# ShuangXieIrene/ssds.pytorch

Measured on AMD Instinct MI355X. Metric: images/sec (fwd+decode+NMS) SSD-MobileNetV2@512, higher is better.
Workload: dtype bf16

## Files before the change

ssds.pytorch_amd/csrc/ssdk_flow_common.h:

```cpp
#pragma once
#include "ssdk_common.h"

namespace ssdk {

typedef __bf16 fl_bf16x8 __attribute__((ext_vector_type(8)));
typedef _Float16 fl_f16x8 __attribute__((ext_vector_type(8)));
typedef float f32x4 __attribute__((ext_vector_type(4)));
typedef _Float16 fl_h2 __attribute__((ext_vector_type(2)));

struct FlowParams {
  const u16* x;
  u16* y;
  const u16* we;
  const float* se;
  const float* be;
  const u16* wd;
  const u16* bd;
  const u16* wp;
  const float* sp;
  const float* bp;
  int N, H, W, Cin, Chid, Cout, Ho, Wo, residual;
  int strips, segs, rs;
  int Himg, Wimg, Cimg, layout;
  unsigned long long seg_mask;
  unsigned long long* dbg;
};

template <int DT>
__device__ __forceinline__ f32x4 fl_mfma(const u32x4& a, const u32x4& b, f32x4 c) {
  if constexpr (DT == SSDK_BF16)
    return __builtin_amdgcn_mfma_f32_16x16x32_bf16(__builtin_bit_cast(fl_bf16x8, a), __builtin_bit_cast(fl_bf16x8, b), c, 0, 0, 0);
  else
    return __builtin_amdgcn_mfma_f32_16x16x32_f16(__builtin_bit_cast(fl_f16x8, a), __builtin_bit_cast(fl_f16x8, b), c, 0, 0, 0);
}
__device__ __forceinline__ fl_h2 fl_as_h2(u32 w) { return __builtin_bit_cast(fl_h2, w); }
__device__ __forceinline__ u32 fl_as_u32(fl_h2 v) { return __builtin_bit_cast(u32, v); }
template <int DT> __device__ __forceinline__ u32 fl_to16(float v) {
  if constexpr (DT == SSDK_BF16) {
    u32 b = __builtin_bit_cast(u32, v);
    if ((b & 0x7fffffffu) > 0x7f800000u) return (b >> 16) | 0x40u;
    return (b + 0x7fffu + ((b >> 16) & 1u)) >> 16;
  } else {
    _Float16 h = (_Float16)v;
    return (u32)__builtin_bit_cast(u16, h);
  }
}
typedef float fl_f32x2 __attribute__((ext_vector_type(2)));
typedef __bf16 fl_bf16x2 __attribute__((ext_vector_type(2)));
template <int DT> __device__ __forceinline__ u32 fl_pack2(float a, float b) {
  const fl_f32x2 v = {a, b};
  if constexpr (DT == SSDK_BF16) return __builtin_bit_cast(u32, __builtin_convertvector(v, fl_bf16x2));
  else return __builtin_bit_cast(u32, __builtin_convertvector(v, fl_h2));
}
template <int DT> __device__ __forceinline__ float fl_from16(u32 h) {
  if constexpr (DT == SSDK_BF16) return bf16_bits_to_f32(h);
  else return f16_bits_to_f32(h);
}
__device__ __forceinline__ u32 fl_from_left(u32 v) { return (u32)__builtin_amdgcn_update_dpp(0, (int)v, 0x111, 0xf, 0xf, true); }
__device__ __forceinline__ u32 fl_from_right(u32 v) { return (u32)__builtin_amdgcn_update_dpp(0, (int)v, 0x101, 0xf, 0xf, true); }

typedef float fl_f2 __attribute__((ext_vector_type(2)));
constexpr float kFlSixth = 1.0f / 6.0f;
__device__ __forceinline__ u32 fl_unit_pack(float a, float b, fl_f2 k) {
  const fl_f2 v = {a, b};
  fl_f2 r;
  asm("v_pk_mul_f32 %0, %1, %2 clamp" : "=v"(r) : "v"(v), "v"(k));
  return __builtin_bit_cast(u32, __builtin_amdgcn_cvt_pkrtz(r[0], r[1]));
}
__device__ __forceinline__ fl_h2 fl_fma_clamp01(fl_h2 a, fl_h2 b, fl_h2 c) {
  fl_h2 r;
  asm("v_pk_fma_f16 %0, %1, %2, %3 clamp" : "=v"(r) : "v"(a), "v"(b), "v"(c));
  return r;
}
__device__ __forceinline__ u32 fl_sixth_h2(u32 w) {
  return fl_to16<SSDK_F16>(fl_from16<SSDK_F16>(w & 0xffffu) * kFlSixth) | (fl_to16<SSDK_F16>(fl_from16<SSDK_F16>(w >> 16) * kFlSixth) << 16);
}

}
```

ssds.pytorch_amd/csrc/ssdk_mbflow.hip:

```cpp
#include <stdio.h>
#include <atomic>
#include <type_traits>

#include "ssdk_common.h"
#include "ssdk_flow_common.h"

namespace ssdk {

constexpr int kFlowThreads = 256;

template <int NCH, int NFO>
struct FlowLds {
  static constexpr int T = (NCH + 1) / 2;
  static constexpr int we = 0;
  static constexpr int sb = we + NCH * 1024;
  static constexpr int wd = sb + NCH * 4 * 32;
  static constexpr int bd = wd + NCH * 9 * 4 * 8;
  static constexpr int wp = (bd + NCH * 4 * 8 + 15) & ~15;
  static constexpr int spb = wp + NFO * T * 1024;
  static constexpr int bytes = spb + NFO * 4 * 32;
};

template <int DT, int S, int NCH, int NFO, int NS, bool STEM = false, bool YE = false, bool PAIR = false, bool XD = false>
__global__ __launch_bounds__(kFlowThreads, ((STEM && !YE) || PAIR) ? 3 : 2) void mbflow_kernel(const FlowParams p) {
  static_assert(!PAIR || (S == 1 && !STEM), "row pairs: stride-1 blocks");
  static_assert(!XD || (STEM && !YE), "dword image loads: the stem's interior instance");
  using L = FlowLds<NCH, NFO>;
  constexpr int T = L::T;
  extern __shared__ __attribute__((aligned(16))) unsigned char smem[];
  const u32 tid = threadIdx.x, lane = tid & 63u, wave = tid >> 6;
  const u32 fr = lane & 15u, fg = lane >> 4;
  const int Cin = p.Cin, Chid = p.Chid, Cout = p.Cout;

  for (u32 i = tid; i < (u32)(NCH * 64); i += kFlowThreads) {
    const u32 c = i >> 6, l = i & 63u, hc = c * 16 + (l & 15u), k0 = (l >> 4) * 8;
    u32x4 v = {0u, 0u, 0u, 0u};
    if constexpr (STEM) {
      if (hc < (u32)Chid) {
#pragma unroll
        for (u32 j = 0; j < 8; ++j) {
          u32 ci, ky, kx;
          bool kv;
          if constexpr (XD) {
            const u32 g = k0 >> 3;
            u32 t;
            if (j < 3u) {
              t = 2u * g;
              kx = j == 2u ? 0u : j + 1u;
              kv = true;
            } else if (j < 6u) {
              t = 2u * g + 1u;
              kx = j == 3u ? 0u : j - 3u;
              kv = true;
            } else {
              t = 8u;
              kx = g == 0u ? j - 5u : 0u;
              kv = g == 0u || (g == 1u && j == 7u);
            }
            ci = t / 3u;
            ky = t % 3u;
            kv = kv && ci < (u32)p.Cimg;
          } else {
            const u32 k = k0 + j;
            ci = k / 9u;
            ky = (k % 9u) / 3u;
            kx = k % 3u;
            kv = k < 27u && ci < (u32)p.Cimg;
          }
          const u32 h = kv ? (u32)p.we[(size_t)hc * 96 + (ky * 8 + kx) * 4 + ci] : 0u;
          v[j >> 1] |= h << ((j & 1u) * 16u);
        }
      }
    } else {
      if (hc < (u32)Chid && k0 < (u32)Cin) v = *reinterpret_cast<const u32x4*>(p.we + (size_t)hc * Cin + k0);
    }
    if (hc < (u32)Chid) {
      const float sc = p.se[hc];
      if (sc != 1.0f) {
#pragma unroll
        for (int q = 0; q < 4; ++q) {
          const u32 w2 = v[q];
          v[q] = fl_to16<DT>(fl_from16<DT>(w2 & 0xffffu) * sc) | (fl_to16<DT>(fl_from16<DT>(w2 >> 16) * sc) << 16);
        }
      }
    }
    *reinterpret_cast<u32x4*>(smem + L::we + i * 16) = v;
  }
  for (u32 i = tid; i < (u32)(NCH * 4); i += kFlowThreads) {
    const u32 hc = (i >> 2) * 16 + (i & 3u) * 4;
    f32x4 s = {0.f, 0.f, 0.f, 0.f}, b = {0.f, 0.f, 0.f, 0.f};
    uint2 d = make_uint2(0u, 0u);
    if (hc < (u32)Chid) {
      s = *reinterpret_cast<const f32x4*>(p.se + hc);
      b = *reinterpret_cast<const f32x4*>(p.be + hc);
      d = *reinterpret_cast<const uint2*>(p.bd + hc);
      d = make_uint2(fl_sixth_h2(d.x), fl_sixth_h2(d.y));
    }
    *reinterpret_cast<f32x4*>(smem + L::sb + i * 32) = s;
    *reinterpret_cast<f32x4*>(smem + L::sb + i * 32 + 16) = b;
    *reinterpret_cast<uint2*>(smem + L::bd + i * 8) = d;
  }
  for (u32 i = tid; i < (u32)(NCH * 9 * 4); i += kFlowThreads) {
    const u32 g = i & 3u, tap = (i >> 2) % 9u, c = (i >> 2) / 9u, hc = c * 16 + g * 4;
    uint2 d = make_uint2(0u, 0u);
    if (hc < (u32)Chid) d = *reinterpret_cast<const uint2*>(p.wd + (size_t)tap * Chid + hc);
    *reinterpret_cast<uint2*>(smem + L::wd + i * 8) = d;
  }
  for (u32 i = tid; i < (u32)(NFO * T * 64 * 2); i += kFlowThreads) {
    const u32 half = i & 1u, l = (i >> 1) & 63u, ft = i >> 7, t = ft % (u32)T, f = ft / (u32)T;
    const u32 co = f * 16 + (l & 15u), hc = (2 * t + half) * 16 + (l >> 4) * 4;
    uint2 d = make_uint2(0u, 0u);
    if (co < (u32)Cout && hc < (u32)Chid) d = *reinterpret_cast<const uint2*>(p.wp + (size_t)co * Chid + hc);
    *reinterpret_cast<uint2*>(smem + L::wp + (ft * 64 + l) * 16 + half * 8) = d;
  }
  for (u32 i = tid; i < (u32)(NFO * 4); i += kFlowThreads) {
    const u32 co = (i >> 2) * 16 + (i & 3u) * 4;
    f32x4 s = {0.f, 0.f, 0.f, 0.f}, b = {0.f, 0.f, 0.f, 0.f};
    if (co < (u32)Cout) {
      s = *reinterpret_cast<const f32x4*>(p.sp + co) * 6.0f;
      b = *reinterpret_cast<const f32x4*>(p.bp + co);
    }
    *reinterpret_cast<f32x4*>(smem + L::spb + i * 32) = s;
    *reinterpret_cast<f32x4*>(smem + L::spb + i * 32 + 16) = b;
  }
  __syncthreads();

  const u32 item = blockIdx.x * (kFlowThreads / 64) + (u32)__builtin_amdgcn_readfirstlane((int)wave);
  const int groups = (p.strips + NS - 1) / NS;
  const int nseg = STEM ? __builtin_popcountll(p.seg_mask) : p.segs;
  const u32 per_img = (u32)(groups * nseg);
  if (item >= (u32)p.N * per_img) return;
  const int n = (int)(item / per_img), rem = (int)(item % per_img);
  int seg = rem / groups;
  const int grp = rem % groups;
  if constexpr (STEM) {
    unsigned long long m = p.seg_mask;
    for (int i = 0; i < seg; ++i) m &= m - 1;
    seg = __builtin_ctzll(m);
  }
  constexpr int OW = S == 1 ? 14 : 7;
  constexpr bool MERGE = S == 2 && NS == 2;
  constexpr int NA = MERGE ? 1 : NS;
  const int oy0 = seg * p.rs, oy1 = (oy0 + p.rs < p.Ho ? oy0 + p.rs : p.Ho) - 1;
  int ix[NS], oxl[NA];
  bool col_ok[NS], out_lane[NA];
#pragma unroll
  for (int s = 0; s < NS; ++s) {
    const int strip = grp * NS + s;
    const int ox0 = strip * OW;
    ix[s] = MERGE ? 2 * (grp * 15 + (int)fr) - s : ox0 * S - 1 + (int)fr;
    col_ok[s] = strip < p.strips && (unsigned)ix[s] < (unsigned)p.W;
    if constexpr (!MERGE) {
      oxl[s] = S == 1 ? ox0 + (int)fr - 1 : ox0 + ((int)fr - 1) / 2;
      out_lane[s] = strip < p.strips && (S == 1 ? (fr >= 1u && fr <= 14u) : ((fr & 1u) && fr <= 13u)) && oxl[s] < p.Wo;
    }
  }
  if constexpr (MERGE) {
    oxl[0] = grp * 15 + (int)fr;
    out_lane[0] = fr <= 14u && oxl[0] < p.Wo;
  }

  const u16* ximg = STEM ? p.x + (size_t)n * p.Cimg * p.Himg * p.Wimg : p.x + (size_t)n * p.H * p.W * Cin;
  const bool k_ok = fg * 8u < (u32)Cin;
  constexpr u32 kOOR = 0x40000000u;
  u32 xoff[STEM ? NS : 1][STEM ? 8 : 1], xoff0[(STEM && !YE) ? NS : 1][(STEM && !YE) ? 8 : 1], kyM[STEM ? 3 : 1];
  const int pstr = STEM ? (p.layout == 1 ? 1 : p.Cimg) : 0, cstr = STEM ? (p.layout == 1 ? p.Himg * p.Wimg : 1) : 0;
  if constexpr (STEM) {
    kyM[0] = kyM[1] = kyM[2] = 0u;
#pragma unroll
    for (int j = 0; j < 8; ++j) {
      const u32 k = fg * 8u + (u32)j, ci = k / 9u, ky = (k % 9u) / 3u, kx = k % 3u;
      const bool kv = k < 27u && ci < (u32)p.Cimg;
      const u32 vo = (u32)(2 * (int)fr * pstr + (int)ci * cstr + ((int)ky * p.Wimg + (int)kx) * pstr) * 2u;
      kyM[0] |= (kv && ky == 0u) ? (1u << j) : 0u;
      kyM[1] |= (kv && ky == 1u) ? (1u << j) : 0u;
      kyM[2] |= (kv && ky == 2u) ? (1u << j) : 0u;
#pragma unroll
      for (int s = 0; s < NS; ++s) {
        xoff[s][j] = (kv && col_ok[s] && (unsigned)(2 * ix[s] - 1 + (int)kx) < (unsigned)p.Wimg) ? vo : kOOR;
        if constexpr (!YE) xoff0[s][j] = ky == 0u ? kOOR : xoff[s][j];
      }
    }
  }
  u32 xd_off[XD ? NS : 1][3], xd_off0[XD ? NS : 1][2], xd_edge[2], xd_edge0[2];
  if constexpr (XD) {
    const u32 tA = 2u * fg, tB = 2u * fg + 1u;
    auto voff = [&](u32 t, int shift, int s_) -> u32 {
      const u32 ci = t / 3u, ky = t % 3u;
      const int px = ix[s_] - shift;
      const bool ok = ci < (u32)p.Cimg && grp * NS + s_ < p.strips && (unsigned)px < (unsigned)p.W;
      return ok ? (u32)((2 * (int)fr + (int)ci * p.Himg * p.Wimg + (int)ky * p.Wimg) * 2 + 4 * (1 - shift)) : kOOR;
    };
#pragma unroll
    for (int s = 0; s < NS; ++s) {
      xd_off[s][0] = voff(tA, 0, s);
      xd_off[s][1] = voff(tB, 0, s);
      xd_off[s][2] = fg == 0u ? voff(8u, 0, s) : (fg == 1u ? voff(8u, 1, s) : kOOR);
      xd_off0[s][0] = tA % 3u == 0u ? kOOR : xd_off[s][0];
      xd_off0[s][1] = tB % 3u == 0u ? kOOR : xd_off[s][1];
    }
    xd_edge[0] = fr == 0u ? voff(tA, 1, 0) : kOOR;
    xd_edge[1] = fr == 0u ? voff(tB, 1, 0) : kOOR;
    xd_edge0[0] = tA % 3u == 0u ? kOOR : xd_edge[0];
    xd_edge0[1] = tB % 3u == 0u ? kOOR : xd_edge[1];
  }
  const int xmargin = STEM ? (p.Wimg + 8) * pstr * 2 : 0;
  const __amdgpu_buffer_rsrc_t xrsrc = __builtin_amdgcn_make_buffer_rsrc(
      (void*)(reinterpret_cast<const unsigned char*>(ximg) - xmargin), 0, STEM ? p.Cimg * p.Himg * p.Wimg * 2 + xmargin : 0, 0x00020000);
  constexpr int XW = STEM ? 8 : 4;
  struct XRow {
    u32 w[XW];
  };
  auto load_x = [&](int iy, int s) -> XRow {
    XRow out;
#pragma unroll
    for (int q = 0; q < XW; ++q) out.w[q] = 0u;
    if constexpr (STEM) {
      const int strip = grp * NS + s;
      const int base = ((2 * iy - 1) * p.Wimg + (2 * (strip * 14 - 1) - 1)) * pstr;
      if constexpr (XD) {
        const bool row_in = (unsigned)iy < (unsigned)p.H, top = iy == 0;
        const int soff = row_in ? (base + 1) * 2 + xmargin - 4 : (int)kOOR;
        out.w[0] = (u32)__builtin_amdgcn_raw_buffer_load_b32(xrsrc, (int)(top ? xd_off0[s][0] : xd_off[s][0]), soff, 0);
        out.w[1] = (u32)__builtin_amdgcn_raw_buffer_load_b32(xrsrc, (int)(top ? xd_off0[s][1] : xd_off[s][1]), soff, 0);
        out.w[2] = (u32)__builtin_amdgcn_raw_buffer_load_b32(xrsrc, (int)xd_off[s][2], soff, 0);
        if (s == 0) {
          out.w[3] = (u32)__builtin_amdgcn_raw_buffer_load_b32(xrsrc, (int)(top ? xd_edge0[0] : xd_edge[0]), soff, 0);
          out.w[4] = (u32)__builtin_amdgcn_raw_buffer_load_b32(xrsrc, (int)(top ? xd_edge0[1] : xd_edge[1]), soff, 0);
        }
        return out;
      } else if constexpr (YE) {
        u32 rowmask = 0;
#pragma unroll
        for (int ky = 0; ky < 3; ++ky)
          rowmask |= ((unsigned)iy < (unsigned)p.H && (unsigned)(2 * iy - 1 + ky) < (unsigned)p.Himg) ? kyM[ky] : 0u;
#pragma unroll
        for (int j = 0; j < 8; ++j) {
          const u32 off = (((rowmask >> j) & 1u) && xoff[s][j] != kOOR) ? xoff[s][j] + (u32)(base * 2 + xmargin) : kOOR;
          out.w[j] = (u32)__builtin_amdgcn_raw_buffer_load_b16(xrsrc, (int)off, 0, 0);
        }
      } else {
        const bool row_in = (unsigned)iy < (unsigned)p.H, top = iy == 0;
        const int soff = row_in ? base * 2 + xmargin : (int)kOOR;
#pragma unroll
        for (int j = 0; j < 8; ++j)
          out.w[j] = (u32)__builtin_amdgcn_raw_buffer_load_b16(xrsrc, (int)(top ? xoff0[s][j] : xoff[s][j]), soff, 0);
      }
      return out;
    } else {
      if (k_ok && col_ok[s] && (unsigned)iy < (unsigned)p.H) {
        const u32x4 v = *reinterpret_cast<const u32x4*>(ximg + ((size_t)iy * p.W + ix[s]) * Cin + fg * 8);
        out.w[0] = v[0];
        out.w[1] = v[1];
        out.w[2] = v[2];
        out.w[3] = v[3];
      }
      return out;
    }
  };

  const bool dbgw = p.dbg != nullptr && blockIdx.x == gridDim.x / 2 && __builtin_amdgcn_readfirstlane((int)wave) == 0;
  int dbg_k = 0;
  fl_h2 accA[NA][NCH * 2], accB[NA][NCH * 2], accC[NA][NCH * 2];
  fl_h2 accD[PAIR ? NA : 1][PAIR ? NCH * 2 : 1];

  auto row = [&](const XRow (&xraw)[NS], int iy, auto FINc, auto MIDc, auto INIc, fl_h2 (&fin)[NA][NCH * 2],
                 fl_h2 (&mid)[NA][NCH * 2], fl_h2 (&ini)[NA][NCH * 2], int oy_fin) {
    constexpr bool FIN = decltype(FINc)::value, MID = decltype(MIDc)::value, INI = decltype(INIc)::value;
    if (dbgw && dbg_k < 250) {
      p.dbg[dbg_k++] = __builtin_readcyclecounter();
      if constexpr (STEM) asm volatile("s_waitcnt vmcnt(16)" ::: "memory");
      else asm volatile("s_waitcnt vmcnt(2)" ::: "memory");
      p.dbg[dbg_k++] = __builtin_readcyclecounter();
    }
    u32x4 xf[NS];
#pragma unroll
    for (int s = 0; s < NS; ++s) {
      if constexpr (XD) {
        int oa, ob;
        if (s == 0) {
          oa = (int)xraw[0].w[3];
          ob = (int)xraw[0].w[4];
        } else {
          oa = __builtin_amdgcn_update_dpp(0, (int)xraw[s - 1].w[0], 0x123, 0xf, 0xf, true);
          ob = __builtin_amdgcn_update_dpp(0, (int)xraw[s - 1].w[1], 0x123, 0xf, 0xf, true);
        }
        const u32 an = (u32)__builtin_amdgcn_update_dpp(oa, (int)xraw[s].w[0], 0x111, 0xf, 0xf, false);
        const u32 bn = (u32)__builtin_amdgcn_update_dpp(ob, (int)xraw[s].w[1], 0x111, 0xf, 0xf, false);
        xf[s][0] = xraw[s].w[0];
        xf[s][1] = __builtin_amdgcn_perm(bn, an, 0x07060302u);
        xf[s][2] = xraw[s].w[1];
        xf[s][3] = fg == 1u ? (xraw[s].w[2] & 0xffff0000u) : xraw[s].w[2];
      } else if constexpr (STEM) {
#pragma unroll
        for (int q = 0; q < 4; ++q) xf[s][q] = xraw[s].w[2 * q] | (xraw[s].w[2 * q + 1] << 16);
      } else {
#pragma unroll
        for (int q = 0; q < 4; ++q) xf[s][q] = xraw[s].w[q];
      }
    }
    fl_f2 hi[NS];
#pragma unroll
    for (int s = 0; s < NS; ++s) {
      const float k = (col_ok[s] && (unsigned)iy < (unsigned)p.H) ? kFlSixth : 0.f;
      hi[s] = fl_f2{k, k};
    }
    const bool store_row = FIN && oy_fin >= oy0 && oy_fin <= oy1;
    uint2 resv[NA][NFO];
    if (!STEM && !MERGE && FIN && store_row && p.residual) {
#pragma unroll
      for (int s = 0; s < NA; ++s)
#pragma unroll
        for (int f = 0; f < NFO; ++f) {
          const int co = f * 16 + (int)fg * 4;
          uint2 r = make_uint2(0u, 0u);
          if (out_lane[s] && co < Cout) r = *reinterpret_cast<const uint2*>(ximg + ((size_t)oy_fin * p.W + oxl[s]) * Cin + co);
          resv[s][f] = r;
        }
    }
    asm volatile("" ::: "memory");
    f32x4 e_cur[NS], e_nxt[NS];
    u32x4 wa = *reinterpret_cast<const u32x4*>(smem + L::we + (int)lane * 16);
    {
      const f32x4 bv0 = *reinterpret_cast<const f32x4*>(smem + L::sb + (int)fg * 32 + 16);
#pragma unroll
      for (int s = 0; s < NS; ++s) e_cur[s] = fl_mfma<DT>(wa, xf[s], bv0);
    }
    if (NCH > 1) wa = *reinterpret_cast<const u32x4*>(smem + L::we + (64 + (int)lane) * 16);
#pragma unroll
    for (int c = 0; c < NCH; ++c) {
      asm volatile("" ::: "memory");
      uint2 wt[9];
#pragma unroll
      for (int t = 0; t < 9; ++t) wt[t] = *reinterpret_cast<const uint2*>(smem + L::wd + ((c * 9 + t) * 4 + (int)fg) * 8);
      uint2 bdi = make_uint2(0u, 0u);
      if constexpr (INI) bdi = *reinterpret_cast<const uint2*>(smem + L::bd + (c * 4 + (int)fg) * 8);
      if (c + 1 < NCH) {
        const f32x4 bvn = *reinterpret_cast<const f32x4*>(smem + L::sb + ((c + 1) * 4 + (int)fg) * 32 + 16);
#pragma unroll
        for (int s = 0; s < NS; ++s) e_nxt[s] = fl_mfma<DT>(wa, xf[s], bvn);
        if (c + 2 < NCH) wa = *reinterpret_cast<const u32x4*>(smem + L::we + ((c + 2) * 64 + (int)lane) * 16);
      }
      __builtin_amdgcn_sched_barrier(0);
      u32 ew[NS][2];
#pragma unroll
      for (int s = 0; s < NS; ++s) {
        const f32x4 e = e_cur[s];
        ew[s][0] = fl_unit_pack(e[0], e[1], hi[s]);
        ew[s][1] = fl_unit_pack(e[2], e[3], hi[s]);
      }
      auto fold = [&](fl_h2 l0, fl_h2 l1, fl_h2 c0, fl_h2 c1, fl_h2 r0, fl_h2 r1, int a) {
        auto taps = [&](int ky, fl_h2& a0, fl_h2& a1, bool init) {
          const uint2 w0 = wt[ky * 3], w1 = wt[ky * 3 + 1], w2 = wt[ky * 3 + 2];
          fl_h2 s0 = init ? fl_as_h2(bdi.x) : a0, s1 = init ? fl_as_h2(bdi.y) : a1;
          s0 = __builtin_elementwise_fma(l0, fl_as_h2(w0.x), s0);
          s1 = __builtin_elementwise_fma(l1, fl_as_h2(w0.y), s1);
          s0 = __builtin_elementwise_fma(c0, fl_as_h2(w1.x), s0);
          s1 = __builtin_elementwise_fma(c1, fl_as_h2(w1.y), s1);
          if (ky == 2) {
            s0 = fl_fma_clamp01(r0, fl_as_h2(w2.x), s0);
            s1 = fl_fma_clamp01(r1, fl_as_h2(w2.y), s1);
          } else {
            s0 = __builtin_elementwise_fma(r0, fl_as_h2(w2.x), s0);
            s1 = __builtin_elementwise_fma(r1, fl_as_h2(w2.y), s1);
          }
          asm volatile("" : "+v"(s0), "+v"(s1));
          a0 = s0;
          a1 = s1;
        };
        if constexpr (INI) taps(0, ini[a][2 * c], ini[a][2 * c + 1], true);
        if constexpr (MID) taps(1, mid[a][2 * c], mid[a][2 * c + 1], false);
        if constexpr (FIN) taps(2, fin[a][2 * c], fin[a][2 * c + 1], false);
      };
      if constexpr (MERGE) {
        fold(fl_as_h2(ew[1][0]), fl_as_h2(ew[1][1]), fl_as_h2(ew[0][0]), fl_as_h2(ew[0][1]), fl_as_h2(fl_from_right(ew[1][0])),
             fl_as_h2(fl_from_right(ew[1][1])), 0);
      } else {
#pragma unroll
        for (int s = 0; s < NS; ++s)
          fold(fl_as_h2(fl_from_left(ew[s][0])), fl_as_h2(fl_from_left(ew[s][1])), fl_as_h2(ew[s][0]), fl_as_h2(ew[s][1]),
               fl_as_h2(fl_from_right(ew[s][0])), fl_as_h2(fl_from_right(ew[s][1])), s);
      }
#pragma unroll
      for (int s = 0; s < NS; ++s) e_cur[s] = e_nxt[s];
      __builtin_amdgcn_sched_barrier(0);
    }
    if (dbgw && dbg_k < 250) p.dbg[dbg_k++] = __builtin_readcyclecounter();
    if constexpr (FIN) {
      if (store_row) {
        asm volatile("" ::: "memory");
        f32x4 yacc[NA][NFO];
#pragma unroll
        for (int s = 0; s < NA; ++s)
#pragma unroll
          for (int f = 0; f < NFO; ++f) yacc[s][f] = f32x4{0.f, 0.f, 0.f, 0.f};
#pragma unroll
        for (int t = 0; t < T; ++t) {
          u32x4 db[NA];
#pragma unroll
          for (int s = 0; s < NA; ++s) {
            db[s][0] = fl_as_u32(fin[s][4 * t]);
            db[s][1] = fl_as_u32(fin[s][4 * t + 1]);
            if (2 * t + 1 < NCH) {
              db[s][2] = fl_as_u32(fin[s][(4 * t + 2 < NCH * 2) ? 4 * t + 2 : 0]);
              db[s][3] = fl_as_u32(fin[s][(4 * t + 3 < NCH * 2) ? 4 * t + 3 : 0]);
            } else {
              db[s][2] = 0u;
              db[s][3] = 0u;
            }
          }
#pragma unroll
          for (int f = 0; f < NFO; ++f) {
            const u32x4 wf = *reinterpret_cast<const u32x4*>(smem + L::wp + ((f * T + t) * 64 + (int)lane) * 16);
#pragma unroll
            for (int s = 0; s < NA; ++s) yacc[s][f] = fl_mfma<SSDK_F16>(wf, db[s], yacc[s][f]);
          }
        }
#pragma unroll
        for (int s = 0; s < NA; ++s) {
          if (out_lane[s]) {
            u16* yrow = p.y + (((size_t)n * p.Ho + oy_fin) * p.Wo + oxl[s]) * Cout;
#pragma unroll
            for (int f = 0; f < NFO; ++f) {
              const int co = f * 16 + (int)fg * 4;
              if (co < Cout) {
                const f32x4 spv = *reinterpret_cast<const f32x4*>(smem + L::spb + (f * 4 + (int)fg) * 32);
                const f32x4 bpv = *reinterpret_cast<const f32x4*>(smem + L::spb + (f * 4 + (int)fg) * 32 + 16);
                u32 h01 = fl_pack2<DT>(fmaf(yacc[s][f][0], spv[0], bpv[0]), fmaf(yacc[s][f][1], spv[1], bpv[1]));
                u32 h23 = fl_pack2<DT>(fmaf(yacc[s][f][2], spv[2], bpv[2]), fmaf(yacc[s][f][3], spv[3], bpv[3]));
                if (!STEM && !MERGE && p.residual) {
                  const u32 x01 = resv[s][f].x, x23 = resv[s][f].y;
                  h01 = fl_pack2<DT>(fl_from16<DT>(h01 & 0xffffu) + fl_from16<DT>(x01 & 0xffffu), fl_from16<DT>(h01 >> 16) + fl_from16<DT>(x01 >> 16));
                  h23 = fl_pack2<DT>(fl_from16<DT>(h23 & 0xffffu) + fl_from16<DT>(x23 & 0xffffu), fl_from16<DT>(h23 >> 16) + fl_from16<DT>(x23 >> 16));
                }
                *reinterpret_cast<uint2*>(yrow + co) = make_uint2(h01, h23);
              }
            }
          }
        }
      }
    }
    if (dbgw && dbg_k < 250) p.dbg[dbg_k++] = __builtin_readcyclecounter();
  };


  auto row2 = [&](const XRow (&x0)[NS], const XRow (&x1)[NS], int iy, fl_h2 (&a0)[NA][NCH * 2], fl_h2 (&a1)[NA][NCH * 2],
                  fl_h2 (&a2)[NA][NCH * 2], fl_h2 (&a3)[NA][NCH * 2]) {
    if (dbgw && dbg_k < 250) {
      p.dbg[dbg_k++] = __builtin_readcyclecounter();
      asm volatile("s_waitcnt vmcnt(4)" ::: "memory");
      p.dbg[dbg_k++] = __builtin_readcyclecounter();
    }
    u32x4 xf[2][NS];
    fl_f2 hi[2][NS];
#pragma unroll
    for (int s = 0; s < NS; ++s) {
#pragma unroll
      for (int q = 0; q < 4; ++q) {
        xf[0][s][q] = x0[s].w[q];
        xf[1][s][q] = x1[s].w[q];
      }
      const float k0 = (col_ok[s] && (unsigned)iy < (unsigned)p.H) ? kFlSixth : 0.f;
      const float k1 = (col_ok[s] && (unsigned)(iy + 1) < (unsigned)p.H) ? kFlSixth : 0.f;
      hi[0][s] = fl_f2{k0, k0};
      hi[1][s] = fl_f2{k1, k1};
    }
    const bool st[2] = {iy - 1 >= oy0 && iy - 1 <= oy1, iy >= oy0 && iy <= oy1};
    uint2 resv[2][NA][NFO];
    if (p.residual) {
#pragma unroll
      for (int o = 0; o < 2; ++o)
#pragma unroll
        for (int s = 0; s < NA; ++s)
#pragma unroll
          for (int f = 0; f < NFO; ++f) {
            const int co = f * 16 + (int)fg * 4;
            uint2 r = make_uint2(0u, 0u);
            if (st[o] && out_lane[s] && co < Cout) r = *reinterpret_cast<const uint2*>(ximg + ((size_t)(iy - 1 + o) * p.W + oxl[s]) * Cin + co);
            resv[o][s][f] = r;
          }
    }
    asm volatile("" ::: "memory");
    f32x4 e_cur[2][NS], e_nxt[2][NS];
    u32x4 wa = *reinterpret_cast<const u32x4*>(smem + L::we + (int)lane * 16);
    {
      const f32x4 bv0 = *reinterpret_cast<const f32x4*>(smem + L::sb + (int)fg * 32 + 16);
#pragma unroll
      for (int o = 0; o < 2; ++o)
#pragma unroll
        for (int s = 0; s < NS; ++s) e_cur[o][s] = fl_mfma<DT>(wa, xf[o][s], bv0);
    }
    if (NCH > 1) wa = *reinterpret_cast<const u32x4*>(smem + L::we + (64 + (int)lane) * 16);
#pragma unroll
    for (int c = 0; c < NCH; ++c) {
      asm volatile("" ::: "memory");
      uint2 wt[9];
#pragma unroll
      for (int t = 0; t < 9; ++t) wt[t] = *reinterpret_cast<const uint2*>(smem + L::wd + ((c * 9 + t) * 4 + (int)fg) * 8);
      const uint2 bdi = *reinterpret_cast<const uint2*>(smem + L::bd + (c * 4 + (int)fg) * 8);
      if (c + 1 < NCH) {
        const f32x4 bvn = *reinterpret_cast<const f32x4*>(smem + L::sb + ((c + 1) * 4 + (int)fg) * 32 + 16);
#pragma unroll
        for (int o = 0; o < 2; ++o)
#pragma unroll
          for (int s = 0; s < NS; ++s) e_nxt[o][s] = fl_mfma<DT>(wa, xf[o][s], bvn);
        if (c + 2 < NCH) wa = *reinterpret_cast<const u32x4*>(smem + L::we + ((c + 2) * 64 + (int)lane) * 16);
      }
      __builtin_amdgcn_sched_barrier(0);
      auto taps = [&](int ky, fl_h2 l0, fl_h2 l1, fl_h2 c0, fl_h2 c1, fl_h2 r0, fl_h2 r1, fl_h2& q0, fl_h2& q1) {
        const uint2 w0 = wt[ky * 3], w1 = wt[ky * 3 + 1], w2 = wt[ky * 3 + 2];
        fl_h2 s0 = ky == 0 ? fl_as_h2(bdi.x) : q0, s1 = ky == 0 ? fl_as_h2(bdi.y) : q1;
        s0 = __builtin_elementwise_fma(l0, fl_as_h2(w0.x), s0);
        s1 = __builtin_elementwise_fma(l1, fl_as_h2(w0.y), s1);
        s0 = __builtin_elementwise_fma(c0, fl_as_h2(w1.x), s0);
        s1 = __builtin_elementwise_fma(c1, fl_as_h2(w1.y), s1);
        if (ky == 2) {
          s0 = fl_fma_clamp01(r0, fl_as_h2(w2.x), s0);
          s1 = fl_fma_clamp01(r1, fl_as_h2(w2.y), s1);
        } else {
          s0 = __builtin_elementwise_fma(r0, fl_as_h2(w2.x), s0);
          s1 = __builtin_elementwise_fma(r1, fl_as_h2(w2.y), s1);
        }
        asm volatile("" : "+v"(s0), "+v"(s1));
        q0 = s0;
        q1 = s1;
      };
#pragma unroll
      for (int o = 0; o < 2; ++o) {
#pragma unroll
        for (int s = 0; s < NS; ++s) {
          const f32x4 e = e_cur[o][s];
          const u32 w0 = fl_unit_pack(e[0], e[1], hi[o][s]), w1 = fl_unit_pack(e[2], e[3], hi[o][s]);
          const fl_h2 l0 = fl_as_h2(fl_from_left(w0)), l1 = fl_as_h2(fl_from_left(w1)), c0 = fl_as_h2(w0), c1 = fl_as_h2(w1);
          const fl_h2 r0 = fl_as_h2(fl_from_right(w0)), r1 = fl_as_h2(fl_from_right(w1));
          if (o == 0) {
            taps(0, l0, l1, c0, c1, r0, r1, a2[s][2 * c], a2[s][2 * c + 1]);
            taps(1, l0, l1, c0, c1, r0, r1, a1[s][2 * c], a1[s][2 * c + 1]);
            taps(2, l0, l1, c0, c1, r0, r1, a0[s][2 * c], a0[s][2 * c + 1]);
          } else {
            taps(0, l0, l1, c0, c1, r0, r1, a3[s][2 * c], a3[s][2 * c + 1]);
            taps(1, l0, l1, c0, c1, r0, r1, a2[s][2 * c], a2[s][2 * c + 1]);
            taps(2, l0, l1, c0, c1, r0, r1, a1[s][2 * c], a1[s][2 * c + 1]);
          }
        }
      }
#pragma unroll
      for (int o = 0; o < 2; ++o)
#pragma unroll
        for (int s = 0; s < NS; ++s) e_cur[o][s] = e_nxt[o][s];
      __builtin_amdgcn_sched_barrier(0);
    }
    if (dbgw && dbg_k < 250) p.dbg[dbg_k++] = __builtin_readcyclecounter();
    if (st[0] || st[1]) {
      asm volatile("" ::: "memory");
      f32x4 yacc[2][NA][NFO];
#pragma unroll
      for (int o = 0; o < 2; ++o)
#pragma unroll
        for (int s = 0; s < NA; ++s)
#pragma unroll
          for (int f = 0; f < NFO; ++f) yacc[o][s][f] = f32x4{0.f, 0.f, 0.f, 0.f};
#pragma unroll
      for (int t = 0; t < T; ++t) {
        u32x4 db[2][NA];
#pragma unroll
        for (int o = 0; o < 2; ++o)
#pragma unroll
          for (int s = 0; s < NA; ++s) {
            const fl_h2* fin = o == 0 ? a0[s] : a1[s];
            db[o][s][0] = fl_as_u32(fin[4 * t]);
            db[o][s][1] = fl_as_u32(fin[4 * t + 1]);
            if (2 * t + 1 < NCH) {
              db[o][s][2] = fl_as_u32(fin[(4 * t + 2 < NCH * 2) ? 4 * t + 2 : 0]);
              db[o][s][3] = fl_as_u32(fin[(4 * t + 3 < NCH * 2) ? 4 * t + 3 : 0]);
            } else {
              db[o][s][2] = 0u;
              db[o][s][3] = 0u;
            }
          }
#pragma unroll
        for (int f = 0; f < NFO; ++f) {
          const u32x4 wf = *reinterpret_cast<const u32x4*>(smem + L::wp + ((f * T + t) * 64 + (int)lane) * 16);
#pragma unroll
          for (int o = 0; o < 2; ++o)
#pragma unroll
            for (int s = 0; s < NA; ++s) yacc[o][s][f] = fl_mfma<SSDK_F16>(wf, db[o][s], yacc[o][s][f]);
        }
      }
#pragma unroll
      for (int f = 0; f < NFO; ++f) {
        const int co = f * 16 + (int)fg * 4;
        if (co < Cout) {
          const f32x4 spv = *reinterpret_cast<const f32x4*>(smem + L::spb + (f * 4 + (int)fg) * 32);
          const f32x4 bpv = *reinterpret_cast<const f32x4*>(smem + L::spb + (f * 4 + (int)fg) * 32 + 16);
#pragma unroll
          for (int o = 0; o < 2; ++o)
#pragma unroll
            for (int s = 0; s < NA; ++s) {
              if (!(st[o] && out_lane[s])) continue;
              u16* yrow = p.y + (((size_t)n * p.Ho + (iy - 1 + o)) * p.Wo + oxl[s]) * Cout;
              u32 h01 = fl_pack2<DT>(fmaf(yacc[o][s][f][0], spv[0], bpv[0]), fmaf(yacc[o][s][f][1], spv[1], bpv[1]));
              u32 h23 = fl_pack2<DT>(fmaf(yacc[o][s][f][2], spv[2], bpv[2]), fmaf(yacc[o][s][f][3], spv[3], bpv[3]));
              if (p.residual) {
                const u32 x01 = resv[o][s][f].x, x23 = resv[o][s][f].y;
                h01 = fl_pack2<DT>(fl_from16<DT>(h01 & 0xffffu) + fl_from16<DT>(x01 & 0xffffu), fl_from16<DT>(h01 >> 16) + fl_from16<DT>(x01 >> 16));
                h23 = fl_pack2<DT>(fl_from16<DT>(h23 & 0xffffu) + fl_from16<DT>(x23 & 0xffffu), fl_from16<DT>(h23 >> 16) + fl_from16<DT>(x23 >> 16));
              }
              *reinterpret_cast<uint2*>(yrow + co) = make_uint2(h01, h23);
            }
        }
      }
    }
    if (dbgw && dbg_k < 250) p.dbg[dbg_k++] = __builtin_readcyclecounter();
  };

  const auto Y = std::true_type{};
  const auto No = std::false_type{};
  auto load_row = [&](XRow (&dst)[NS], int iy) {
#pragma unroll
    for (int s = 0; s < NS; ++s) dst[s] = load_x(iy, s);
  };
  XRow xa[NS], xb[NS];
  {
    if constexpr (PAIR) {
      const int rend = oy1 + 1;
      XRow xc[NS], xd[NS];
      load_row(xa, oy0 - 1);
      load_row(xb, oy0);
      for (int r = oy0 - 1; r <= rend; r += 4) {
        load_row(xc, r + 2);
        load_row(xd, r + 3);
        row2(xa, xb, r, accA, accB, accC, accD);
        load_row(xa, r + 4);
        load_row(xb, r + 5);
        row2(xc, xd, r + 2, accC, accD, accA, accB);
      }
    } else if constexpr (S == 1) {
      const int rend = oy1 + 1;
      load_row(xa, oy0 - 1);
      for (int r = oy0 - 1; r <= rend; r += 6) {
        load_row(xb, r + 1);
        row(xa, r, Y, Y, Y, accA, accB, accC, r - 1);
        load_row(xa, r + 2);
        row(xb, r + 1, Y, Y, Y, accB, accC, accA, r);
        load_row(xb, r + 3);
        row(xa, r + 2, Y, Y, Y, accC, accA, accB, r + 1);
        load_row(xa, r + 4);
        row(xb, r + 3, Y, Y, Y, accA, accB, accC, r + 2);
        load_row(xb, r + 5);
        row(xa, r + 4, Y, Y, Y, accB, accC, accA, r + 3);
        load_row(xa, r + 6);
        row(xb, r + 5, Y, Y, Y, accC, accA, accB, r + 4);
      }
    } else {
      const int rend = 2 * oy1 + 1;
      load_row(xa, 2 * oy0 - 1);
      for (int r = 2 * oy0 - 1; r <= rend; r += 4) {
        load_row(xb, r + 1);
        row(xa, r, Y, No, Y, accA, accC, accB, (r - 1) / 2);
        load_row(xa, r + 2);
        row(xb, r + 1, No, Y, No, accC, accB, accC, 0);
        load_row(xb, r + 3);
        row(xa, r + 2, Y, No, Y, accB, accC, accA, (r + 1) / 2);
        load_row(xa, r + 4);
        row(xb, r + 3, No, Y, No, accC, accA, accC, 0);
      }
    }
  }
}

constexpr int kFlowNS = 2;

template <int DT, int S, int NCH, int NFO>
static void flow_launch(const FlowParams& p, unsigned grid, hipStream_t stream) {
  constexpr int lds = FlowLds<NCH, NFO>::bytes;
  if constexpr (S == 1 && NCH == 9) {
    if (p.layout == 101) {
      static const int pair = getenv("SSDK_FLOW_PAIR") ? atoi(getenv("SSDK_FLOW_PAIR")) : 1;
      if (pair) {
        (void)hipFuncSetAttribute(reinterpret_cast<const void*>(&mbflow_kernel<DT, S, NCH, NFO, 1, false, false, true>), hipFuncAttributeMaxDynamicSharedMemorySize, lds);
        hipLaunchKernelGGL((mbflow_kernel<DT, S, NCH, NFO, 1, false, false, true>), dim3(grid), dim3(kFlowThreads), lds, stream, p);
        return;
      }
      (void)hipFuncSetAttribute(reinterpret_cast<const void*>(&mbflow_kernel<DT, S, NCH, NFO, 1>), hipFuncAttributeMaxDynamicSharedMemorySize, lds);
      hipLaunchKernelGGL((mbflow_kernel<DT, S, NCH, NFO, 1>), dim3(grid), dim3(kFlowThreads), lds, stream, p);
      return;
    }
  }
  (void)hipFuncSetAttribute(reinterpret_cast<const void*>(&mbflow_kernel<DT, S, NCH, NFO, kFlowNS>), hipFuncAttributeMaxDynamicSharedMemorySize, lds);
  hipLaunchKernelGGL((mbflow_kernel<DT, S, NCH, NFO, kFlowNS>), dim3(grid), dim3(kFlowThreads), lds, stream, p);
}

template <int DT, int S>
static bool flow_dispatch(const FlowParams& p, int nch, int nfo, unsigned grid, hipStream_t stream) {
#define SSDK_FLOW(NCH_, NFO_)                                   \
  if (nch == NCH_ && nfo == NFO_) {                             \
    flow_launch<DT, S, NCH_, NFO_>(p, grid, stream);            \
    return true;                                                \
  }
  SSDK_FLOW(6, 2)
  SSDK_FLOW(9, 2)
  SSDK_FLOW(12, 2)
  SSDK_FLOW(12, 4)
#undef SSDK_FLOW
  return false;
}

int launch_mbflow(const ssdk_mbconv_desc* d, hipStream_t stream) {
  static const int env = getenv("SSDK_MB_FLOW") ? atoi(getenv("SSDK_MB_FLOW")) : 1;
  const int variant = d->variant;
  if ((!env && variant <= 0) || variant < 0 || variant == 2 || variant == 3) return 1;
  const bool stem = d->stem != 0;
  if (stem) {
    if (d->Cin > 3 || d->Chid != 32 || d->Cout != 16 || d->stride != 1 || d->residual) return 1;
  } else if (d->Cin > 32 || (d->Cin % 8) || d->Chid > 192 || (d->Chid % 16) || d->Cout > 64 || (d->Cout % 8)) {
    return 1;
  }
  const int nch = d->Chid / 16, nfo = stem ? 1 : (d->Cout <= 32 ? 2 : 4);
  if (!stem && !((nch == 6 || nch == 9 || nch == 12) && (nfo == 2 || nch == 12))) return 1;
  FlowParams p;
  p.x = (const u16*)d->x;
  p.y = (u16*)d->y;
  p.we = (const u16*)d->w_expand;
  p.se = d->scale_expand;
  p.be = d->bias_expand;
  p.wd = (const u16*)d->w_dw;
  p.bd = (const u16*)d->bias_dw;
  p.wp = (const u16*)d->w_project;
  p.sp = d->scale_project;
  p.bp = d->bias_project;
  p.N = d->N;
  p.H = d->H;
  p.W = d->W;
  p.Cin = d->Cin;
  p.Himg = d->H;
  p.Wimg = d->W;
  p.Cimg = d->Cin;
  p.layout = d->stem;
  if (stem) {
    p.H = (d->H + 2 - 3) / 2 + 1;
    p.W = (d->W + 2 - 3) / 2 + 1;
    p.Cin = 32;
  }
  p.Chid = d->Chid;
  p.Cout = d->Cout;
  p.Ho = (p.H + 2 - 3) / d->stride + 1;
  p.Wo = (p.W + 2 - 3) / d->stride + 1;
  p.residual = d->residual;
  p.seg_mask = 0;
  p.dbg = nullptr;
  static const int env_dbg = getenv("SSDK_MB_DBG") ? atoi(getenv("SSDK_MB_DBG")) : 0;
  static unsigned long long* dbg_dev = nullptr;
  if (env_dbg) {
    if (!dbg_dev) (void)hipMalloc(&dbg_dev, 256 * sizeof(unsigned long long));
    (void)hipMemsetAsync(dbg_dev, 0, 256 * sizeof(unsigned long long), stream);
    p.dbg = dbg_dev;
  }
  auto dbg_print = [&]() {
    if (!env_dbg) return;
    unsigned long long hh[256];
    (void)hipStreamSynchronize(stream);
    (void)hipMemcpy(hh, dbg_dev, sizeof(hh), hipMemcpyDeviceToHost);
    fprintf(stderr, "[mbflow dbg] Cin=%d Chid=%d Cout=%d s=%d stem=%d rs=%d: per row (wait x | chunks | project+store | to next row):", d->Cin,
            d->Chid, d->Cout, d->stride, (int)stem, p.rs);
    for (int i = 0; i + 4 < 250 && hh[i + 4]; i += 4)
      fprintf(stderr, " [%llu %llu %llu %llu]", hh[i + 1] - hh[i], hh[i + 2] - hh[i + 1], hh[i + 3] - hh[i + 2], hh[i + 4] - hh[i + 3]);
    fprintf(stderr, "\n");
  };
  const int ow = d->stride == 1 ? 14 : 7;
  p.strips = (p.Wo + ow - 1) / ow;
  if (d->stride == 2) p.strips = 2 * ((p.Wo + 14) / 15);
  constexpr int env_rs = 0;
  constexpr int env_ns1 = 1;
  const bool ns1 = ((env_ns1 & 1) && !stem && d->stride == 1 && nch == 9) || ((env_ns1 & 2) && stem);
  const int flow_ns = ns1 ? 1 : kFlowNS;
  if (ns1 && !stem) p.layout = 101;
  const int groups = (p.strips + flow_ns - 1) / flow_ns;
  int rs = 64;
  while (rs > 16 && (long)d->N * groups * ((p.Ho + rs - 1) / rs) < 4096) rs >>= 1;
  if ((long)d->N * groups * ((p.Ho + rs - 1) / rs) < 2048 && env_rs <= 0 && variant <= 0) return 1;
  if (variant > 0) {
    while (rs > 8 && (long)d->N * groups * ((p.Ho + rs - 1) / rs) < 2048) rs >>= 1;
  }
  if (env_rs > 0) rs = env_rs;
  if (rs > p.Ho) rs = p.Ho;
  p.rs = rs;
  p.segs = (p.Ho + rs - 1) / rs;
  const long items = (long)d->N * groups * p.segs;
  const unsigned grid = (unsigned)((items + 3) / 4);
  bool ok;
  if (stem) {
    if (p.segs > 64) return 1;
    unsigned long long edge = 0;
    for (int sgi = 0; sgi < p.segs; ++sgi) {
      const int o0 = sgi * p.rs, o1 = (o0 + p.rs < p.Ho ? o0 + p.rs : p.Ho) - 1;
      const int last_row = o1 + 1 < p.H - 1 ? o1 + 1 : p.H - 1;
      if (2 * last_row + 1 >= p.Himg) edge |= 1ull << sgi;
    }
    const unsigned long long all = p.segs == 64 ? ~0ull : ((1ull << p.segs) - 1ull);
    constexpr int lds = FlowLds<2, 1>::bytes;
    auto go = [&](auto DTc, auto YEc, unsigned long long mask) {
      constexpr int DTv = decltype(DTc)::value;
      constexpr bool YEv = decltype(YEc)::value;
      if (!mask) return;
      FlowParams q = p;
      q.seg_mask = mask;
      const long it = (long)d->N * groups * __builtin_popcountll(mask);
      const unsigned g = (unsigned)((it + 3) / 4);
      if (ns1) {
        (void)hipFuncSetAttribute(reinterpret_cast<const void*>(&mbflow_kernel<DTv, 1, 2, 1, 1, true, YEv>),
                                  hipFuncAttributeMaxDynamicSharedMemorySize, lds);
        hipLaunchKernelGGL((mbflow_kernel<DTv, 1, 2, 1, 1, true, YEv>), dim3(g), dim3(kFlowThreads), lds, stream, q);
        return;
      }
      if constexpr (!YEv) {
        static const int env_xd = getenv("SSDK_STEM_DWORD") ? atoi(getenv("SSDK_STEM_DWORD")) : 1;
        if (env_xd && q.layout == 1 && (q.Wimg & 1) == 0 && (reinterpret_cast<uintptr_t>(q.x) & 3u) == 0) {
          (void)hipFuncSetAttribute(reinterpret_cast<const void*>(&mbflow_kernel<DTv, 1, 2, 1, kFlowNS, true, false, false, true>),
                                    hipFuncAttributeMaxDynamicSharedMemorySize, lds);
          hipLaunchKernelGGL((mbflow_kernel<DTv, 1, 2, 1, kFlowNS, true, false, false, true>), dim3(g), dim3(kFlowThreads), lds, stream, q);
          return;
        }
      }
      (void)hipFuncSetAttribute(reinterpret_cast<const void*>(&mbflow_kernel<DTv, 1, 2, 1, kFlowNS, true, YEv>),
                                hipFuncAttributeMaxDynamicSharedMemorySize, lds);
      hipLaunchKernelGGL((mbflow_kernel<DTv, 1, 2, 1, kFlowNS, true, YEv>), dim3(g), dim3(kFlowThreads), lds, stream, q);
    };
    if (d->dtype == SSDK_BF16) {
      go(std::integral_constant<int, SSDK_BF16>{}, std::false_type{}, all & ~edge);
      go(std::integral_constant<int, SSDK_BF16>{}, std::true_type{}, edge);
    } else {
      go(std::integral_constant<int, SSDK_F16>{}, std::false_type{}, all & ~edge);
      go(std::integral_constant<int, SSDK_F16>{}, std::true_type{}, edge);
    }
    dbg_print();
    return 0;
  }
  if (d->dtype == SSDK_BF16) ok = d->stride == 1 ? flow_dispatch<SSDK_BF16, 1>(p, nch, nfo, grid, stream) : flow_dispatch<SSDK_BF16, 2>(p, nch, nfo, grid, stream);
  else ok = d->stride == 1 ? flow_dispatch<SSDK_F16, 1>(p, nch, nfo, grid, stream) : flow_dispatch<SSDK_F16, 2>(p, nch, nfo, grid, stream);
  if (ok) dbg_print();
  return ok ? 0 : 1;
}

}
```

Before: 64060.

## Plan row-segment split per layer with a CU-aware load-balance cost model

Swaps the fixed power-of-two row-segment size for a host-side planner. It searches segment splits of two different sizes, scores each by the worst per-wave-slot row visits given the CU count, and picks the cheapest. The kernel learns to decode two segment sizes and an optional segment-major item ordering. Plans are cached per shape, and the intent is to reduce tail imbalance and wasted halo rows across CUs. The cost is a mutex lookup on every launch, and the model may not match real scheduling.

Result: no change. 64410, median of 5 (+0.5%).

```diff
diff --git a/ssds.pytorch_amd/csrc/ssdk_flow_common.h b/ssds.pytorch_amd/csrc/ssdk_flow_common.h
--- a/ssds.pytorch_amd/csrc/ssdk_flow_common.h
+++ b/ssds.pytorch_amd/csrc/ssdk_flow_common.h
@@ -21,6 +21,7 @@
   const float* bp;
   int N, H, W, Cin, Chid, Cout, Ho, Wo, residual;
   int strips, segs, rs;
+  int segs_a = 0, rs_b = 0, seg_major = 0;
   int Himg, Wimg, Cimg, layout;
   unsigned long long seg_mask;
   unsigned long long* dbg;
diff --git a/ssds.pytorch_amd/csrc/ssdk_flow_plan.h b/ssds.pytorch_amd/csrc/ssdk_flow_plan.h
--- /dev/null
+++ b/ssds.pytorch_amd/csrc/ssdk_flow_plan.h
@@ -0,0 +1,96 @@
+#pragma once
+#include <vector>
+
+namespace ssdk {
+
+enum FlowLoop {
+  kFlowLoopS1 = 0,
+  kFlowLoopPair = 1,
+  kFlowLoopS2 = 2,
+};
+
+struct FlowPlan {
+  int rs_a, n_a, rs_b, n_b;
+  int seg_major;
+  long long cost;
+  long long rows;
+  long long items;
+};
+
+inline int flow_item_visits(int rows, int loop) {
+  const int need = loop == kFlowLoopS2 ? 2 * rows + 1 : rows + 2, step = loop == kFlowLoopS1 ? 6 : 4;
+  return (need + step - 1) / step * step;
+}
+
+inline long long flow_layout_cost(const std::vector<int>& seg_rows, int N, int groups, int loop, int waves, int cus, bool seg_major) {
+  const long long nseg = (long long)seg_rows.size(), per_seg = (long long)N * groups, items = per_seg * nseg;
+  std::vector<long long> slot((size_t)waves * cus, 0);
+  long long worst = 0;
+  for (long long i = 0; i < items; ++i) {
+    const int seg = (int)(seg_major ? i / per_seg : (i % ((long long)groups * nseg)) / groups);
+    long long& s = slot[(size_t)(i % ((long long)waves * cus))];
+    s += flow_item_visits(seg_rows[(size_t)seg], loop);
+    if (s > worst) worst = s;
+  }
+  return worst;
+}
+
+inline std::vector<int> flow_plan_segments(const FlowPlan& pl) {
+  std::vector<int> v((size_t)pl.n_a, pl.rs_a);
+  v.insert(v.end(), (size_t)pl.n_b, pl.rs_b);
+  return v;
+}
+
+inline bool flow_plan_too_small(int N, int Ho, int groups) { return (long long)N * groups * ((Ho + 15) / 16) < 2048; }
+
+inline FlowPlan flow_plan(int N, int Ho, int groups, int loop, int waves, int cus, int max_segs) {
+  const long long per_seg = (long long)N * groups, slots = (long long)waves * cus;
+  FlowPlan best{};
+  bool have = false;
+  auto consider = [&](int rs_a, int n_a, int rs_b, int n_b) {
+    if (max_segs > 0 && n_a + n_b > max_segs) return;
+    const int va = flow_item_visits(rs_a, loop), vb = n_b ? flow_item_visits(rs_b, loop) : va;
+    FlowPlan c{rs_a, n_a, n_b ? rs_b : rs_a, n_b, va != vb, 0, 0, 0};
+    c.items = per_seg * (n_a + n_b);
+    c.rows = per_seg * ((long long)n_a * va + (long long)n_b * vb);
+    for (long long i = 0; i < c.items; i += slots) c.cost += i / per_seg < n_a ? va : vb;
+    if (!have || c.cost < best.cost || (c.cost == best.cost && (c.rows < best.rows || (c.rows == best.rows && c.items > best.items)))) {
+      best = c;
+      have = true;
+    }
+  };
+  if (Ho < 8) consider(Ho, 1, Ho, 0);
+  for (int rs_a = 8; rs_a <= Ho; ++rs_a) {
+    for (int n_a = 1; n_a * rs_a <= Ho; ++n_a) {
+      const int rest = Ho - n_a * rs_a;
+      if (rest == 0) {
+        consider(rs_a, n_a, rs_a, 0);
+        continue;
+      }
+      if (rest < rs_a) consider(rs_a, n_a, rest, 1);
+      for (int n_b = 2; n_b * 8 <= rest; ++n_b)
+        if (rest % n_b == 0 && rest / n_b < rs_a) consider(rs_a, n_a, rest / n_b, n_b);
+    }
+  }
+  return best;
+}
+
+inline FlowPlan flow_plan_rule(int N, int Ho, int groups, int loop, int waves, int cus) {
+  int rs = 64;
+  while (rs > 16 && (long long)N * groups * ((Ho + rs - 1) / rs) < 4096) rs >>= 1;
+  if (rs > Ho) rs = Ho;
+  const int rest = Ho % rs;
+  FlowPlan p{rs, Ho / rs, rest ? rest : rs, rest ? 1 : 0, 0, 0, 0, 0};
+  const std::vector<int> seg = flow_plan_segments(p);
+  p.items = (long long)N * groups * (long long)seg.size();
+  for (int r : seg) p.rows += (long long)N * groups * flow_item_visits(r, loop);
+  p.cost = flow_layout_cost(seg, N, groups, loop, waves, cus, false);
+  return p;
+}
+
+inline FlowPlan flow_plan_launch(int N, int Ho, int groups, int loop, int waves, int cus, int max_segs) {
+  if (loop == kFlowLoopPair) return flow_plan_rule(N, Ho, groups, loop, waves, cus);
+  return flow_plan(N, Ho, groups, loop, waves, cus, max_segs);
+}
+
+}
diff --git a/ssds.pytorch_amd/csrc/ssdk_mbflow.hip b/ssds.pytorch_amd/csrc/ssdk_mbflow.hip
--- a/ssds.pytorch_amd/csrc/ssdk_mbflow.hip
+++ b/ssds.pytorch_amd/csrc/ssdk_mbflow.hip
@@ -1,9 +1,13 @@
 #include <stdio.h>
+#include <algorithm>
 #include <atomic>
+#include <mutex>
 #include <type_traits>
+#include <vector>
 
 #include "ssdk_common.h"
 #include "ssdk_flow_common.h"
+#include "ssdk_flow_plan.h"
 
 namespace ssdk {
 
@@ -130,8 +134,10 @@
   const int nseg = STEM ? __builtin_popcountll(p.seg_mask) : p.segs;
   const u32 per_img = (u32)(groups * nseg);
   if (item >= (u32)p.N * per_img) return;
-  const int n = (int)(item / per_img), rem = (int)(item % per_img);
-  int seg = rem / groups;
+  const u32 per_seg = (u32)(p.N * groups);
+  const int rem = (int)(p.seg_major ? item % per_seg : item % per_img);
+  const int n = p.seg_major ? rem / groups : (int)(item / per_img);
+  int seg = p.seg_major ? (int)(item / per_seg) : rem / groups;
   const int grp = rem % groups;
   if constexpr (STEM) {
     unsigned long long m = p.seg_mask;
@@ -141,7 +147,9 @@
   constexpr int OW = S == 1 ? 14 : 7;
   constexpr bool MERGE = S == 2 && NS == 2;
   constexpr int NA = MERGE ? 1 : NS;
-  const int oy0 = seg * p.rs, oy1 = (oy0 + p.rs < p.Ho ? oy0 + p.rs : p.Ho) - 1;
+  const bool seg_a = seg < p.segs_a;
+  const int oy0 = seg_a ? seg * p.rs : p.segs_a * p.rs + (seg - p.segs_a) * p.rs_b, seg_rows = seg_a ? p.rs : p.rs_b;
+  const int oy1 = (oy0 + seg_rows < p.Ho ? oy0 + seg_rows : p.Ho) - 1;
   int ix[NS], oxl[NA];
   bool col_ok[NS], out_lane[NA];
 #pragma unroll
@@ -706,6 +714,37 @@
   return false;
 }
 
+static int flow_cu_count() {
+  constexpr int kMaxDev = 64;
+  static std::atomic<int> cus_of[kMaxDev];
+  int dev = 0;
+  if (hipGetDevice(&dev) != hipSuccess || dev < 0 || dev >= kMaxDev) return 0;
+  int cus = cus_of[dev].load(std::memory_order_relaxed);
+  if (!cus) {
+    if (hipDeviceGetAttribute(&cus, hipDeviceAttributeMultiprocessorCount, dev) != hipSuccess || cus <= 0) return 0;
+    cus_of[dev].store(cus, std::memory_order_relaxed);
+  }
+  return cus;
+}
+
+static FlowPlan flow_plan_cached(int N, int Ho, int groups, int loop, int cus, int max_segs) {
+  struct Entry {
+    int key[6];
+    FlowPlan plan;
+  };
+  static std::mutex mu;
+  static std::vector<Entry> seen;
+  const int key[6] = {N, Ho, groups, loop, cus, max_segs};
+  std::lock_guard<std::mutex> lock(mu);
+  for (const Entry& e : seen)
+    if (std::equal(key, key + 6, e.key)) return e.plan;
+  Entry e;
+  std::copy(key, key + 6, e.key);
+  e.plan = flow_plan_launch(N, Ho, groups, loop, kFlowThreads / 64, cus, max_segs);
+  seen.push_back(e);
+  return e.plan;
+}
+
 int launch_mbflow(const ssdk_mbconv_desc* d, hipStream_t stream) {
   static const int env = getenv("SSDK_MB_FLOW") ? atoi(getenv("SSDK_MB_FLOW")) : 1;
   const int variant = d->variant;
@@ -770,22 +809,30 @@
   const int ow = d->stride == 1 ? 14 : 7;
   p.strips = (p.Wo + ow - 1) / ow;
   if (d->stride == 2) p.strips = 2 * ((p.Wo + 14) / 15);
-  constexpr int env_rs = 0;
   constexpr int env_ns1 = 1;
   const bool ns1 = ((env_ns1 & 1) && !stem && d->stride == 1 && nch == 9) || ((env_ns1 & 2) && stem);
   const int flow_ns = ns1 ? 1 : kFlowNS;
   if (ns1 && !stem) p.layout = 101;
   const int groups = (p.strips + flow_ns - 1) / flow_ns;
-  int rs = 64;
-  while (rs > 16 && (long)d->N * groups * ((p.Ho + rs - 1) / rs) < 4096) rs >>= 1;
-  if ((long)d->N * groups * ((p.Ho + rs - 1) / rs) < 2048 && env_rs <= 0 && variant <= 0) return 1;
   if (variant > 0) {
-    while (rs > 8 && (long)d->N * groups * ((p.Ho + rs - 1) / rs) < 2048) rs >>= 1;
-  }
-  if (env_rs > 0) rs = env_rs;
-  if (rs > p.Ho) rs = p.Ho;
-  p.rs = rs;
-  p.segs = (p.Ho + rs - 1) / rs;
+    int rs = 64;
+    while (rs > 8 && (long)d->N * groups * ((p.Ho + rs - 1) / rs) < (rs > 16 ? 4096 : 2048)) rs >>= 1;
+    if (rs > p.Ho) rs = p.Ho;
+    p.rs = p.rs_b = rs;
+    p.segs = p.segs_a = (p.Ho + rs - 1) / rs;
+    p.seg_major = 0;
+  } else {
+    if (flow_plan_too_small(d->N, p.Ho, groups)) return 1;
+    const int cus = flow_cu_count();
+    if (cus <= 0) return 1;
+    const int loop = d->stride == 2 ? kFlowLoopS2 : (ns1 && !stem ? kFlowLoopPair : kFlowLoopS1);
+    const FlowPlan pl = flow_plan_cached(d->N, p.Ho, groups, loop, cus, stem ? 64 : 0);
+    p.rs = pl.rs_a;
+    p.segs_a = pl.n_a;
+    p.rs_b = pl.rs_b;
+    p.segs = pl.n_a + pl.n_b;
+    p.seg_major = pl.seg_major;
+  }
   const long items = (long)d->N * groups * p.segs;
   const unsigned grid = (unsigned)((items + 3) / 4);
   bool ok;
@@ -793,7 +840,8 @@
     if (p.segs > 64) return 1;
     unsigned long long edge = 0;
     for (int sgi = 0; sgi < p.segs; ++sgi) {
-      const int o0 = sgi * p.rs, o1 = (o0 + p.rs < p.Ho ? o0 + p.rs : p.Ho) - 1;
+      const int o0 = sgi < p.segs_a ? sgi * p.rs : p.segs_a * p.rs + (sgi - p.segs_a) * p.rs_b, len = sgi < p.segs_a ? p.rs : p.rs_b;
+      const int o1 = (o0 + len < p.Ho ? o0 + len : p.Ho) - 1;
       const int last_row = o1 + 1 < p.H - 1 ? o1 + 1 : p.H - 1;
       if (2 * last_row + 1 >= p.Himg) edge |= 1ull << sgi;
     }
```
